# XunshanMan/MVGFormer

Measured on AMD Instinct MI355X. Metric: decoder samples/sec (5-view, 1024 queries, 4 layers), higher is better.
Workload: dtype bf16; 1 GPU; cfg2: 5 views, 1024 queries x 15 joints, 4 decoder layers, maps [(128, 240), (64, 120), (32, 60)] x 256ch, all queries valid; parallelism=single GPU, pyramid_handoff=NCHW fp32 (reference producer format), packed per step, initial_poses='sample_space' grid over the whole space (SURVEY 8(d)), samples_in_flight=1, samples_per_forward=1, hip_graph=True, device=gfx950:sramecc+:xnack-, cus=256

## Files before the change

### include/mvg_decoder.h

```cpp
#ifndef MVG_DECODER_H
#define MVG_DECODER_H

#include <stddef.h>
#include <stdint.h>

#ifdef __cplusplus
extern "C" {
#endif

#define MVG_F32 0
#define MVG_BF16 1

#define MVG_E_BADARG 10001
#define MVG_E_NOGPU 10002

#define MVG_CAM_STRIDE 48

int mvg_device_info(char* arch_out, int arch_len, int* cu_count);
const char* mvg_version(void);
int mvg_set_tuning(const char* key, int value);

int mvg_msda_forward_f32(const float* value, const int64_t* spatial_shapes,
                         const int64_t* level_start_index, const float* sampling_loc,
                         const float* attn_weight, float* out,
// ... 74 lines not shown
int mvg_msda_fused(const void* value, int dtype, const float* oa, const float* ref_lvl,
                   const int64_t* shapes_host, const int64_t* starts_host, void* samp,
                   int N_img, int Lq, int L, int S, void* stream);

int mvg_msda_gfused_f32(const float* value, const float* G, const float* xw, const float* ref_lvl,
                        const int64_t* shapes_host, const int64_t* starts_host, float* samp,
                        const uint8_t* pair_mask, const int32_t* order,
                        int N_img, int Lq, int L, int S, int B, void* stream);

int mvg_pyramid_group_ws(const void* feat, int n_img, int S, int njobs, const void* const* Wf, const float* const* bias,
                         void* const* out, const int* N, const int* planes, int slots_per_xcd, void* stream);
int mvg_msda_gsamp(const void* vh, const void* G, const float* xw, const float* ref_lvl,
                   const int64_t* shapes_host, const int64_t* starts_host, void* samp,
                   const uint8_t* pair_mask, const int32_t* order,
                   int N_img, int Lq, int L, int S, int B, void* stream);

size_t mvg_bin_pairs_workspace(int N_img, int Lq);
int mvg_bin_pairs(const float* ref_lvl, const uint8_t* inside, const int64_t* shapes_host, int L, int32_t* order,
                  int N_img, int Lq, void* workspace, size_t workspace_bytes, void* stream);

int mvg_mean_views(const void* attn, int dtype, void* out, int V, int rows, int C, void* stream);

int mvg_add_layernorm(const float* res, const void* h, int h_dtype, const float* gamma,
                      const float* beta, float* y, int rows, int C, void* stream);

int mvg_class_head(const float* tgt, const float* Wc, const float* bc, float threshold,
                   const uint8_t* forced_valid, float* prob, uint8_t* valid, int* any_valid,
                   int B, int NQ, int J, int C, void* stream);

int mvg_rowdot3(const void* h, int h_dtype, const float* W3, const float* b3, float* o,
                int rows, int C, void* stream);

int mvg_chain_attn_pose(const void* samp, const uint8_t* inside, const void* Wp, const float* bp,
                        const void* W0, const float* b0, const void* W1, const float* b1,
// ... 109 lines not shown
```

### mvgformer_amd/_lib.py

```python
from __future__ import annotations

import ctypes as C
import os

import torch

_HERE = os.path.dirname(os.path.abspath(__file__))
LIB_PATH = os.environ.get("MVG_LIB") or os.path.join(_HERE, "libmvgformer_hip.so")

MVG_F32, MVG_BF16 = 0, 1
CAM_STRIDE = 48

_vp, _i, _f = C.c_void_p, C.c_int, C.c_float

SIGNATURES = {
    "mvg_device_info": [C.c_char_p, _i, C.POINTER(_i)],
    "mvg_set_tuning": [C.c_char_p, _i],
    "mvg_msda_forward_f32": [_vp] * 6 + [_i] * 7 + [_vp],
    "mvg_msda_forward_bf16": [_vp] * 6 + [_i] * 7 + [_vp],
    "mvg_msda_backward_f32": [_vp] * 9 + [_i] * 7 + [_vp],
    "mvg_msda_backward_det_workspace": [_i] * 7 + [_vp],
    "mvg_msda_backward_det_f32": [_vp] * 9 + [_i] * 7 + [_vp, C.c_size_t, _vp],
    "mvg_msda_backward_det_bf16": [_vp] * 9 + [_i] * 7 + [_vp, C.c_size_t, _vp],
    "mvg_msda_backward_bal_workspace": [_i] * 7 + [_vp, _i],
# ... 9 lines not shown
    "mvg_dlt_backward": [_vp, _vp, _vp, _vp, _vp, _vp, _vp, _i, _i, _i, _i, _vp],
    "mvg_linear_wgrad_bias_f32": [_vp, _i, _vp, _i, _vp, _vp, _vp, _vp, _i, _i, _i, _i, _vp],
    "mvg_linear_wgrad_bias_bf16": [_vp, _i, _vp, _i, _vp, _vp, _vp, _vp, _i, _i, _i, _i, _vp],
    "mvg_linear_ordered": [_vp, _i, _vp, _vp, _vp, _i, _vp, _i, _i, _i, _i, _vp, _vp, _vp, _vp],
    "mvg_linear_sum": [_vp, _vp, _i, _i, _vp, _i, _vp, _vp, _i, _i, _vp, _i, _i, _i, _i, _vp],
    "mvg_msda_fused": [_vp, _i, _vp, _vp, _vp, _vp, _vp, _i, _i, _i, _i, _vp],
    "mvg_msda_gfused_f32": [_vp] * 9 + [_i] * 5 + [_vp],
    "mvg_chain_attn_pose": [_vp] * 14 + [_i, _vp],
    "mvg_chain_update_ffn_class": [_vp, _i] + [_vp] * 13 + [_f] + [_vp] * 9 + [_i] * 5 + [_vp, _vp],
    "mvg_chain_update_ffn_class_f32h": [_vp, _i, _vp, _vp, _i, _vp, _vp, _vp, _vp, _i, _vp, _vp, _i, _vp, _vp, _vp, _vp, _vp, C.c_float, _vp,
                                        _vp, _vp, _vp, _vp, _vp, _vp, _i, _vp, _vp, _i, _i, _i, _i, _i, _vp],
    "mvg_chain_attn_pose_f32h": [_vp, _vp, _vp, _i, _vp, _vp, _i, _vp, _vp, _i, _vp, _vp, _vp, _vp, _vp, _vp, _vp, _i, _vp],
    "mvg_pyramid_f32h": [_vp, _vp, _i, _vp, _vp, _i, _vp, _vp, C.c_int64, _i, _vp],
    "mvg_pyramid_group_ws": [_vp, _i, _i, _i, _vp, _vp, _vp, _vp, _vp, _i, _vp],
    "mvg_msda_gsamp": [_vp] * 9 + [_i] * 5 + [_vp],
    "mvg_bin_pairs": [_vp] * 3 + [_i] + [_vp] + [_i] * 2 + [_vp, C.c_size_t, _vp],
    "mvg_bin_pairs_workspace": [_i, _i],
    "mvg_mean_views": [_vp, _i, _vp, _i, _i, _i, _vp],
    "mvg_add_layernorm": [_vp, _vp, _i, _vp, _vp, _vp, _i, _i, _vp],
    "mvg_class_head": [_vp, _vp, _vp, _f, _vp, _vp, _vp, _vp, _i, _i, _i, _i, _vp],
    "mvg_rowdot3": [_vp, _i, _vp, _vp, _vp, _i, _i, _vp],
    "mvg_triangulate": [_vp] * 8 + [_i] * 4 + [_vp],
    "mvg_triangulate_project": [_vp] * 8 + [_i] * 4 + [_vp, _i] + [_vp] * 4,
    "mvg_uncrop_undistort_jac": [_vp, _vp, _vp, _vp, _i, _i, _i, _vp],
    "mvg_sym4_eigh": [_vp] * 3 + [C.c_long, _vp],
    "mvg_knn_match_workspace": [_i] * 3,
    "mvg_knn_match": [_vp, _vp, _vp, _i, _vp, _vp, _i, _i, _f] + [_i] * 5 + [_vp, C.c_size_t] + [_vp] * 5,
    "mvg_knn_match_jm": [_vp, _vp, _vp, _i, _vp, _vp, _i, _i, _f] + [_i] * 5 + [_vp, _i, _vp, C.c_size_t] + [_vp] * 5,
    "mvg_criterion_workspace": [_i] * 5,
    "mvg_criterion": [_vp] * 10 + [_i] + [_vp] * 4 + [_f] * 3 + [_i] * 7 + [_vp, C.c_size_t] + [_vp] * 5,
    "mvg_criterion_jm": [_vp] * 10 + [_i] + [_vp] * 4 + [_f] * 3 + [_i] * 5 + [_vp] + [_i] * 3 + [_vp, C.c_size_t] + [_vp] * 5,
# ... 91 lines not shown
```

### mvgformer_amd/csrc/geom.hip

```cpp
#include "common.h"

template <typename T>
__device__ __forceinline__ void pack_tile(const float* __restrict__ src, T* __restrict__ feat, int C, int HW, int S, int start,
                                          int bx, float (&tile)[64][65]) {
  const int n = blockIdx.z, tid = threadIdx.x;
  const int hw0 = bx * 64, c0 = blockIdx.y * 64;
  const int tx = tid & 63, ty = tid >> 6;
  const float* sp = src + (long)n * C * HW;
  float v[16];
#pragma unroll
  for (int i = 0; i < 16; ++i) {
    const int c = min(c0 + ty + 4 * i, C - 1), hw = min(hw0 + tx, HW - 1);
    v[i] = sp[(long)c * HW + hw];
  }
#pragma unroll
  for (int i = 0; i < 16; ++i) tile[ty + 4 * i][tx] = v[i];
  __syncthreads();
  T* fp = feat + ((long)n * S + start) * C;
  const int cq = tid & 15, p = tid >> 4, c = c0 + 4 * cq;
  const bool vec = (C & 3) == 0;
#pragma unroll
  for (int i = 0; i < 4; ++i) {
    const int hw = hw0 + p + 16 * i;
    if (hw >= HW || c >= C) continue;
// ... 768 lines not shown

constexpr int BIN_BITS = 6, BIN_KEYS = 1 << (2 * BIN_BITS);

__device__ __forceinline__ unsigned spread1(unsigned v) {
  v &= 0x3fu;
  v = (v | (v << 8)) & 0x00ff00ffu;
  v = (v | (v << 4)) & 0x0f0f0f0fu;
  v = (v | (v << 2)) & 0x33333333u;
  v = (v | (v << 1)) & 0x55555555u;
  return v;
}

template <int KPT>
__global__ __launch_bounds__(1024) void bin_pairs_kernel(const float* __restrict__ ref_lvl,
                                                         const uint8_t* __restrict__ inside, int* __restrict__ order,
                                                         int Lq, int L, int W0, int H0, int shift) {
  __shared__ int hist[BIN_KEYS + 1];
  __shared__ int wave_tot[16];
  const int n = blockIdx.x, tid = threadIdx.x;
  for (int i = tid; i <= BIN_KEYS; i += 1024) hist[i] = 0;
  float rx[KPT], ry[KPT];
  uint8_t in[KPT];
#pragma unroll
  for (int k = 0; k < KPT; ++k) {
    const long pair = (long)n * Lq + min(tid + 1024 * k, Lq - 1);
    const float2 rr = *reinterpret_cast<const float2*>(ref_lvl + pair * L * 2);
    rx[k] = rr.x;
    ry[k] = rr.y;
    in[k] = inside ? inside[pair] : (uint8_t)1;
  }
  __syncthreads();
  int key[KPT];
#pragma unroll
  for (int k = 0; k < KPT; ++k) {
    const int cx = min(max((int)(fminf(fmaxf(rx[k], 0.f), 1.f) * (float)W0), 0), W0 - 1) >> shift;
    const int cy = min(max((int)(fminf(fmaxf(ry[k], 0.f), 1.f) * (float)H0), 0), H0 - 1) >> shift;
    key[k] = in[k] ? (int)(spread1((unsigned)cx) | (spread1((unsigned)cy) << 1)) : BIN_KEYS;
    const bool live = tid + 1024 * k < Lq;
    const unsigned long long outm = __ballot(live && key[k] == BIN_KEYS);
    if (live && key[k] != BIN_KEYS) atomicAdd(&hist[key[k]], 1);
    if (outm && (tid & 63) == 0) atomicAdd(&hist[BIN_KEYS], __popcll(outm));
  }
  __syncthreads();
  const int c0 = hist[4 * tid], c1 = hist[4 * tid + 1], c2 = hist[4 * tid + 2], c3 = hist[4 * tid + 3];
  const int mine = c0 + c1 + c2 + c3;
  int incl = mine;
#pragma unroll
  for (int d = 1; d < 64; d <<= 1) {
    const int up = __shfl_up(incl, d, 64);
    if ((tid & 63) >= d) incl += up;
  }
  if ((tid & 63) == 63) wave_tot[tid >> 6] = incl;
  __syncthreads();
  int base = 0, total = 0;
#pragma unroll
  for (int w = 0; w < 16; ++w) {
    const int t = wave_tot[w];
    base += (w < (tid >> 6)) ? t : 0;
    total += t;
  }
  __syncthreads();
  const int ex = base + incl - mine;
  hist[4 * tid] = ex;
  hist[4 * tid + 1] = ex + c0;
  hist[4 * tid + 2] = ex + c0 + c1;
  hist[4 * tid + 3] = ex + c0 + c1 + c2;
  if (tid == 0) hist[BIN_KEYS] = total;
  __syncthreads();
#pragma unroll
  for (int k = 0; k < KPT; ++k) {
    const bool live = tid + 1024 * k < Lq;
    const bool out = live && key[k] == BIN_KEYS;
    const unsigned long long outm = __ballot(out);
    int pos = 0;
    if (live && !out) pos = atomicAdd(&hist[key[k]], 1);
    int obase = 0;
    if (outm && (tid & 63) == 0) obase = atomicAdd(&hist[BIN_KEYS], __popcll(outm));
    obase = __shfl(obase, 0, 64);
    if (out) pos = obase + __popcll(outm & ((1ull << (tid & 63)) - 1ull));
    if (live) order[(long)n * Lq + pos] = n * Lq + tid + 1024 * k;
  }
}

int g_bin_multi = 1;
constexpr int BIN_PARTS = 8;
constexpr int BIN_MULTI_MIN = 8192;
constexpr int BIN_CNT_STRIDE = BIN_KEYS + 4;

template <int KPT>
__global__ __launch_bounds__(1024) void bin_count_kernel(const float* __restrict__ ref_lvl,
                                                         const uint8_t* __restrict__ inside, unsigned* __restrict__ cnt,
                                                         unsigned short* __restrict__ keys_out, int Lq, int Lp, int L,
                                                         int W0, int H0, int shift) {
  __shared__ int hist[BIN_KEYS + 4];
  const int n = blockIdx.x / BIN_PARTS, part = blockIdx.x % BIN_PARTS, tid = threadIdx.x;
// ... 18 lines not shown
    const bool live = tid + 1024 * k < nq;
    const unsigned long long outm = __ballot(live && key == BIN_KEYS);
    if (live && key != BIN_KEYS) atomicAdd(&hist[key], 1);
    if (outm && (tid & 63) == 0) atomicAdd(&hist[BIN_KEYS], __popcll(outm));
    if (live) keys_out[(long)n * Lq + q0 + tid + 1024 * k] = (unsigned short)key;
  }
  __syncthreads();
  unsigned* dst = cnt + (long)blockIdx.x * BIN_CNT_STRIDE;
  *reinterpret_cast<uint4*>(dst + 4 * tid) = *reinterpret_cast<const uint4*>(&hist[4 * tid]);
  if (tid == 0) *reinterpret_cast<uint4*>(dst + BIN_KEYS) = *reinterpret_cast<const uint4*>(&hist[BIN_KEYS]);
}

template <int KPT>
__global__ __launch_bounds__(1024) void bin_scatter_kernel(const unsigned* __restrict__ cnt,
                                                           const unsigned short* __restrict__ keys_in,
                                                           int* __restrict__ order, int Lq, int Lp) {
  __shared__ int hist[BIN_KEYS + 4];
  __shared__ int wave_tot[16];
  __shared__ int out_sums[2];
  const int n = blockIdx.x / BIN_PARTS, part = blockIdx.x % BIN_PARTS, tid = threadIdx.x;
  const int n_img = gridDim.x / BIN_PARTS;
  constexpr int OVN = 16;
  int ov[OVN];
  if (tid < 64) {
#pragma unroll
    for (int j = 0; j < OVN; ++j) {
      const int i = tid + 64 * j;
      ov[j] = i < n_img * BIN_PARTS ? (int)cnt[(long)i * BIN_CNT_STRIDE + BIN_KEYS] : 0;
    }
  }
  const int q0 = part * Lp, nq = max(0, min(Lp, Lq - q0));
// ... 30 lines not shown
      ob += ((tid + 64 * j) / BIN_PARTS < n) ? ov[j] : 0;
    }
    for (int i = tid + 64 * OVN; i < n_img * BIN_PARTS; i += 64) {
      const int v = (int)cnt[(long)i * BIN_CNT_STRIDE + BIN_KEYS];
      oa += v;
      ob += (i / BIN_PARTS < n) ? v : 0;
    }
#pragma unroll
    for (int off = 32; off > 0; off >>= 1) {
      ob += __shfl_xor(ob, off, 64);
      oa += __shfl_xor(oa, off, 64);
    }
    if (tid == 0) {
      out_sums[0] = ob;
      out_sums[1] = oa;
    }
  }
  __syncthreads();
  int base = 0, total = 0;
#pragma unroll
  for (int w = 0; w < 16; ++w) {
    const int t = wave_tot[w];
    base += (w < (tid >> 6)) ? t : 0;
    total += t;
  }
  const int ex = base + incl - mine;
  hist[4 * tid] = ex + before[0];
  hist[4 * tid + 1] = ex + tot[0] + before[1];
  hist[4 * tid + 2] = ex + tot[0] + tot[1] + before[2];
  hist[4 * tid + 3] = ex + tot[0] + tot[1] + tot[2] + before[3];
// ... 307 lines not shown
  int e = mvg_fill_levels(&lv, shapes_host, zeros, L);
  if (e) return e;
  const long total = (long)V * B * Lq;
  if (total == 0) return 0;
  hipLaunchKernelGGL(project_kernel, dim3(mvg_ceil_div(total, 256)), dim3(256), 0, (hipStream_t)stream, X, cams, lv, r,
                     ref_lvl, inside, B, Lq, total);
  MVG_LAUNCH_CHECK();
  return 0;
}

size_t mvg_bin_pairs_workspace(int N_img, int Lq) {
  if (N_img <= 0 || Lq < BIN_MULTI_MIN) return 0;
  return (size_t)N_img * BIN_PARTS * BIN_CNT_STRIDE * sizeof(unsigned) + (size_t)N_img * Lq * sizeof(unsigned short);
}

int mvg_bin_pairs(const float* ref_lvl, const uint8_t* inside, const int64_t* shapes_host, int L, int32_t* order,
                  int N_img, int Lq, void* workspace, size_t workspace_bytes, void* stream) {
  if (!ref_lvl || !shapes_host || !order || L <= 0 || N_img < 0 || Lq < 0) return MVG_E_BADARG;
  if ((long)N_img * Lq > 0x7fffffffL) return MVG_E_BADARG;
  if (N_img == 0 || Lq == 0) return 0;
  const int H0 = (int)shapes_host[0], W0 = (int)shapes_host[1];
  if (H0 <= 0 || W0 <= 0) return MVG_E_BADARG;
  int shift = 2;
  while (((W0 - 1) >> shift) >= (1 << BIN_BITS) || ((H0 - 1) >> shift) >= (1 << BIN_BITS)) ++shift;
  if (Lq > 64 * 1024) return MVG_E_BADARG;
  hipStream_t st = (hipStream_t)stream;
  if (g_bin_multi && Lq >= BIN_MULTI_MIN && workspace && workspace_bytes >= mvg_bin_pairs_workspace(N_img, Lq)) {
    unsigned* cnt = reinterpret_cast<unsigned*>(workspace);
    unsigned short* keys = reinterpret_cast<unsigned short*>(cnt + (size_t)N_img * BIN_PARTS * BIN_CNT_STRIDE);
    const int Lp = ((Lq + BIN_PARTS - 1) / BIN_PARTS + 63) / 64 * 64;
#define MVG_BIN2(K)                                                                                              \
  {                                                                                                              \
    hipLaunchKernelGGL((bin_count_kernel<K>), dim3(N_img * BIN_PARTS), dim3(1024), 0, st, ref_lvl, inside, cnt,  \
                       keys, Lq, Lp, L, W0, H0, shift);                                                          \
    hipLaunchKernelGGL((bin_scatter_kernel<K>), dim3(N_img * BIN_PARTS), dim3(1024), 0, st, cnt, keys,           \
                       (int*)order, Lq, Lp);                                                                     \
  }
    if (Lp <= 1024) MVG_BIN2(1)
    else if (Lp <= 2 * 1024) MVG_BIN2(2)
    else if (Lp <= 4 * 1024) MVG_BIN2(4)
    else MVG_BIN2(8)
#undef MVG_BIN2
    MVG_LAUNCH_CHECK();
    return 0;
  }
#define MVG_BIN(K)                                                                                               \
  hipLaunchKernelGGL((bin_pairs_kernel<K>), dim3(N_img), dim3(1024), 0, st, ref_lvl, inside,                     \
                     (int*)order, Lq, L, W0, H0, shift)
  if (Lq <= 2 * 1024) MVG_BIN(2);
  else if (Lq <= 4 * 1024) MVG_BIN(4);
  else if (Lq <= 8 * 1024) MVG_BIN(8);
  else if (Lq <= 16 * 1024) MVG_BIN(16);
  else if (Lq <= 32 * 1024) MVG_BIN(32);
  else MVG_BIN(64);
#undef MVG_BIN
  MVG_LAUNCH_CHECK();
  return 0;
}

int mvg_gather_ref(const void* feat, int dtype, const float* ref_lvl, const float* x, const int64_t* shapes_host,
                   const int64_t* starts_host, void* ain, int V, int B, int Lq, int L, int S, int C, void* stream) {
  if (!feat || !ref_lvl || !x || !shapes_host || !starts_host || !ain || C % 4 != 0) return MVG_E_BADARG;
  LevelTable lv;
  int e = mvg_fill_levels(&lv, shapes_host, starts_host, L);
  if (e) return e;
  const long pairs = (long)V * B * Lq;
  if (pairs == 0) return 0;
  const int grid = mvg_ceil_div(pairs, 4);
  if (dtype == MVG_F32)
    hipLaunchKernelGGL((gather_ref_kernel<float>), dim3(grid), dim3(256), 0, (hipStream_t)stream, (const float*)feat, ref_lvl, x,
                       lv, (float*)ain, B, Lq, S, C, (int)pairs);
  else if (dtype == MVG_BF16)
// ... 139 lines not shown
```

### mvgformer_amd/csrc/msda.hip

```cpp
#include <string.h>

#include "common.h"
#include "gsamp_dev.h"


template <typename T>
__device__ __forceinline__ f32x4 bilinear4(const T* __restrict__ lvl_base, int H, int W, long row_stride,
                                           float h_im, float w_im, float scale) {
  const bool inside = (h_im > -1.f) && (w_im > -1.f) && (h_im < (float)H) && (w_im < (float)W);
  h_im = index_safe(h_im, (float)H);
  w_im = index_safe(w_im, (float)W);
  const float hl_f = floorf(h_im), wl_f = floorf(w_im);
  const int h_low = (int)hl_f, w_low = (int)wl_f;
  const int h_high = h_low + 1, w_high = w_low + 1;
  const float lh = h_im - hl_f, lw = w_im - wl_f;
  const float hh = 1.f - lh, hw = 1.f - lw;
  const float s = inside ? scale : 0.f;
  const bool hl_ok = h_low >= 0, hh_ok = h_high <= H - 1, wl_ok = w_low >= 0, wh_ok = w_high <= W - 1;
  const float w1 = (hl_ok && wl_ok) ? hh * hw : 0.f;
  const float w2 = (hl_ok && wh_ok) ? hh * lw : 0.f;
  const float w3 = (hh_ok && wl_ok) ? lh * hw : 0.f;
  const float w4 = (hh_ok && wh_ok) ? lh * lw : 0.f;
  const int hl_c = min(max(h_low, 0), H - 1), hh_c = min(max(h_high, 0), H - 1);
  const int wl_c = min(max(w_low, 0), W - 1), wh_c = min(max(w_high, 0), W - 1);
// ... 721 lines not shown
  if (reset) {
    const unsigned z = 0;
    e = hipMemcpyToSymbol(HIP_SYMBOL(gsamp_stamp_count), &z, sizeof(z));
    if (e != hipSuccess) return -(int)e;
  }
  return (int)n;
}
#endif

template <int L, int NT, int PIPE = 0>
__device__ __forceinline__ void msda_gsamp_body(const bf16_t* __restrict__ vp, const bf16_t* __restrict__ G,
                                                const float* __restrict__ xw, const float* __restrict__ r,
                                                const LevelTable& lv, bf16_t* __restrict__ samp,
                                                const uint8_t* __restrict__ pair_mask,
                                                const int* __restrict__ order, int n_pairs,
                                                int Lq, int S, int B, int map_ch) {
  constexpr int SCP = 3 * L * 8 + 8;
  __shared__ __attribute__((aligned(16))) float scratch[NT / 64][16][SCP];
  const int wave = threadIdx.x >> 6, lane = threadIdx.x & 63;
  const int sub = lane & 3, pl = lane >> 2;
  int m, pblk;
  if (map_ch == 0) {
    m = blockIdx.x & 7;
    pblk = blockIdx.x >> 3;
  } else {
    const int xcd = blockIdx.x & 7, j = blockIdx.x >> 3;
    m = j & 7;
    const int t = j >> 3;
    pblk = ((t / map_ch) * 8 + xcd) * map_ch + t % map_ch;
  }
  const int slot = pblk * (NT / 4) + wave * 16 + pl;
#ifdef GSAMP_STAMPS
  const unsigned long long gs_t0 = __builtin_amdgcn_s_memrealtime();
  auto gs_flush = [&](bool sampled) {
    const unsigned long long act = __ballot(sampled);
    const int first = __ffsll((unsigned long long)__ballot(true)) - 1;
    if (wave == 0 && lane == first) {
      const unsigned s_ = atomicAdd(&gsamp_stamp_count, 1u);
      if (s_ < 65536) {
        unsigned hw, xcc;
        asm volatile("s_getreg_b32 %0, hwreg(HW_REG_HW_ID)" : "=s"(hw));
        asm volatile("s_getreg_b32 %0, hwreg(HW_REG_XCC_ID)" : "=s"(xcc));
        gsamp_stamps[s_ * 4] = blockIdx.x | ((unsigned long long)__popcll(act) << 32);
        gsamp_stamps[s_ * 4 + 1] = gs_t0;
// ... 21 lines not shown
    }
  }
  float acc[8];
  gsamp_unit<L, PIPE>(vp, G, xw, r, lv, &scratch[wave][pl][0], pair, m, sub, Lq, S, B, acc, mine);
  store_acc<bf16_t, 8>(samp + (long)pair * 256 + m * 32 + sub * 8, acc);
#ifdef GSAMP_STAMPS
  gs_flush(true);
#endif
}

template <int L, int NT>
__global__ __launch_bounds__(NT) void msda_gsamp_kernel(const bf16_t* __restrict__ vp, const bf16_t* __restrict__ G,
                                                        const float* __restrict__ xw, const float* __restrict__ r,
                                                        LevelTable lv, bf16_t* __restrict__ samp,
                                                        const uint8_t* __restrict__ pair_mask, const int* __restrict__ order,
                                                        int n_pairs, int Lq, int S, int B, int map_ch) {
  msda_gsamp_body<L, NT>(vp, G, xw, r, lv, samp, pair_mask, order, n_pairs, Lq, S, B, map_ch);
}
template <int L, int NT>
__global__ __launch_bounds__(NT) void msda_gsamp_pipe_kernel(const bf16_t* __restrict__ vp, const bf16_t* __restrict__ G,
                                                             const float* __restrict__ xw, const float* __restrict__ r,
                                                             LevelTable lv, bf16_t* __restrict__ samp,
                                                             const uint8_t* __restrict__ pair_mask, const int* __restrict__ order,
                                                             int n_pairs, int Lq, int S, int B, int map_ch) {
  msda_gsamp_body<L, NT, 1>(vp, G, xw, r, lv, samp, pair_mask, order, n_pairs, Lq, S, B, map_ch);
}

static int g_gsamp_pipe = 0;
int g_auto_small = 1;
static int g_gsamp_map = 4;
static int g_gfused_chunk = 4;
static int g_gsamp_lds_pad = 0;
static int g_gsamp_threads = 256;

template <typename T, int CPL, int NB>
static int launch_msda_fused_cpl(const T* value, const float* oa, const float* r, const LevelTable& lv, T* samp,
                                 int n_pairs, int Lq, int S, hipStream_t st) {
  constexpr int PPW = CPL / 4;
  const int grid = (n_pairs + 4 * PPW - 1) / (4 * PPW);
  switch (lv.L) {
// ... 180 lines not shown
    case 32: MVG_BWD(32); break;
    case 64: MVG_BWD(64); break;
    default: {
      hipError_t e = hipMemsetAsync(grad_sampling_loc, 0, sizeof(float) * (size_t)N * Lq * M * L * P * 2, st);
      if (e != hipSuccess) return (int)e;
      e = hipMemsetAsync(grad_attn_weight, 0, sizeof(float) * (size_t)N * Lq * M * L * P, st);
      if (e != hipSuccess) return (int)e;
      MVG_BWD(0);
    }
  }
#undef MVG_BWD
  MVG_LAUNCH_CHECK();
  return 0;
}

int mvg_msda_gsamp(const void* vp, const void* G, const float* xw, const float* ref_lvl, const int64_t* shapes_host,
                   const int64_t* starts_host, void* samp, const uint8_t* pair_mask, const int32_t* order, int N_img,
                   int Lq, int L, int S, int B, void* stream) {
  if (!vp || !G || !xw || !ref_lvl || !shapes_host || !starts_host || !samp || B <= 0) return MVG_E_BADARG;
  LevelTable lv;
  int e = mvg_fill_levels(&lv, shapes_host, starts_host, L);
  if (e) return e;
  const long pairs = (long)N_img * Lq;
  if (pairs > 0x7fffffffL / 4) return MVG_E_BADARG;
  if ((long)N_img * S * 384 >= 0xffffffffL || (long)N_img * 8 * S * 64 >= 0xffffffffL) return MVG_E_BADARG;
  if (pairs == 0) return 0;
  hipStream_t st = (hipStream_t)stream;
  const bool pipe = g_gsamp_pipe == 1 || (g_gsamp_pipe == 0 && (long)N_img * Lq >= 32768);
  int nthreads = g_gsamp_threads, map = g_gsamp_map;
  if (g_auto_small && Lq <= 8192) {
    nthreads = 128;
    map = 1;
  }
#define MVG_GS(LL, NT)                                                                                            \
  {                                                                                                               \
    int npb = (int)((pairs + NT / 4 - 1) / (NT / 4));                                                             \
    if (map > 0) npb = (npb + 8 * map - 1) / (8 * map) * (8 * map);                                               \
    if (pipe)                                                                                                 \
      hipLaunchKernelGGL((msda_gsamp_pipe_kernel<LL, NT>), dim3(8 * npb), dim3(NT), g_gsamp_lds_pad, st, (const bf16_t*)vp,     \
                         (const bf16_t*)G, xw, ref_lvl, lv, (bf16_t*)samp, pair_mask, order, (int)pairs, Lq, S,   \
                         B, map);                                                                                 \
    else                                                                                                          \
      hipLaunchKernelGGL((msda_gsamp_kernel<LL, NT>), dim3(8 * npb), dim3(NT), g_gsamp_lds_pad, st, (const bf16_t*)vp,          \
                         (const bf16_t*)G, xw, ref_lvl, lv, (bf16_t*)samp, pair_mask, order, (int)pairs, Lq, S,   \
                         B, map);                                                                                 \
  }
#define MVG_GSN(LL)                                                                                               \
  if (nthreads == 1024) MVG_GS(LL, 1024) else if (nthreads == 512) MVG_GS(LL, 512)                                \
  else if (nthreads == 128) MVG_GS(LL, 128) else MVG_GS(LL, 256)
  switch (L) {
    case 1: MVG_GSN(1); break;
    case 2: MVG_GSN(2); break;
    case 3: MVG_GSN(3); break;
    case 4: MVG_GSN(4); break;
    default: return MVG_E_BADARG;
  }
#undef MVG_GSN
#undef MVG_GS
  MVG_LAUNCH_CHECK();
  return 0;
}

extern int g_chain_rm;
extern int g_chain_a_lds_pad;
extern int g_linear_tiles;
extern int g_f32_split;
extern int g_wreg_grid;
extern int g_f32h_rows;
extern int g_bin_multi;

int mvg_set_tuning(const char* key, int value) {
  if (!key) return MVG_E_BADARG;
  if (!strcmp(key, "linear_tiles") && value >= 0 && value <= 2) { g_linear_tiles = value; return 0; }
  if (!strcmp(key, "f32_split") && (value == 0 || value == 1)) { g_f32_split = value; return 0; }
  if (!strcmp(key, "f32h_rows") && (value == 0 || value == 32 || value == 64)) { g_f32h_rows = value; return 0; }
// ... 60 lines not shown
```

### mvgformer_amd/decoder.py

```python
from __future__ import annotations

import copy
import os

import torch
import torch.nn.functional as F
from torch import nn

from . import ops
from .projattn import ProjAttn, WeightCache



class MLP(nn.Module):

    def __init__(self, input_dim, hidden_dim, output_dim, num_layers):
        super().__init__()
        self.num_layers = num_layers
        h = [hidden_dim] * (num_layers - 1)
        self.layers = nn.ModuleList(nn.Linear(n, k) for n, k in zip([input_dim] + h, h + [output_dim]))

    def forward(self, x):
        for i, layer in enumerate(self.layers):
            x = F.relu(layer(x)) if i < self.num_layers - 1 else layer(x)
# ... 148 lines not shown
        self.use_confidences = False
        self.class_embed = nn.Linear(d_model, 2)
        self.num_joints = num_joints
        self.feature_update_method = feature_update_method
        self.init_self_attention = init_self_attention
        self.open_forward_ffn = open_forward_ffn
        self.query_filter_method = query_filter_method
        self.visualization_jump_num = visualization_jump_num
        self.triangulation_method = triangulation_method
        self.filter_query = filter_query
        self.d_model = d_model
        self.compute_dtype = torch.float32
        self.training_dtype = torch.float32
        self.use_fused_chains = True
        self.use_fused_chains_f32 = os.environ.get("MVG_F32_FUSED", "1") != "0"
        self.fuse_boundary = True
        self.skip_masked_f32 = True
        self._wc = WeightCache()
        self._run = None
        self._any_valid_hook = None

    def set_compute_dtype(self, dtype):
        if dtype not in (torch.float32, torch.bfloat16):
            raise ValueError("compute dtype must be float32 or bfloat16")
        self.compute_dtype = dtype
        self.proj_attn.compute_dtype = dtype
        return self

    def set_training_dtype(self, dtype):
        if dtype not in (torch.float32, torch.bfloat16):
# ... 308 lines not shown
        if xw_in is not None and tuple(xw_in.shape) != (B * Lq, 192):
            xw_in = None
        f32 = torch.float32
        pose_layers = self.pose_embed.MLP.layers
        o = None
        if self.proj_attn._vp_event is None and getattr(ctx, "_packed_event", None) is not None:
            torch.cuda.current_stream().wait_event(ctx._packed_event)
            ctx.feat.record_stream(torch.cuda.current_stream())
        if path_a == "bf16":
            order = None
            mode = self.proj_attn.sort_pairs if Lq <= 65536 else False
            if mode == "first":
                if getattr(ctx, "order", None) is None or ctx.order.numel() != V * B * Lq:
                    ctx.order = ops.bin_pairs(ref_lvl, None, ctx.levels)
                order = ctx.order
            elif mode:
                order = ops.bin_pairs(ref_lvl, inside.view(-1), ctx.levels)
            samp = self.proj_attn.native_sample(x, ref_lvl, ctx.feat, ctx.levels, V, B, pair_mask=inside.view(-1),
                                                order=order, xw=xw_in)
            wts, o_masked = self._chain_a_weights(dt)
            attn, o = ops.chain_attn_pose(samp, inside.view(-1), *wts, order=order, o_masked=o_masked)
        elif path_a == "f32h":
            order = ops.bin_pairs(ref_lvl, inside.view(-1), ctx.levels) if (self.proj_attn.sort_pairs and Lq <= 65536) else None
            samp = self.proj_attn.native_sample(x, ref_lvl, ctx.feat, ctx.levels, V, B, pair_mask=inside.view(-1), order=order,
                                                xw=xw_in)
            wts, o_masked = self._chain_a_weights_f32h()
            attn, o = ops.chain_attn_pose_f32h(samp, inside.view(-1), *wts, order=order, o_masked=o_masked)
        else:
            order32 = None
            if (dt == torch.float32 and self.skip_masked_f32 and C == 256 and 8192 <= Lq <= 65536
                    and self.proj_attn.sort_pairs):
                order32 = ops.bin_pairs(ref_lvl, inside.view(-1), ctx.levels)
            attn = self.proj_attn.native_forward(x(), ref_lvl, ctx.feat, ctx.levels, V, B, rowmask=inside.view(-1), order=order32)

        forced = None
# ... 306 lines not shown
```

### mvgformer_amd/ops.py

```python
from __future__ import annotations

import ctypes as C

import math

import numpy as np
import torch

from . import _lib as L

BACKWARD_MODE = __import__("os").environ.get("MVG_BACKWARD", "det")
BACKWARD_CHUNK = None


def _det_entry(lib, bf16, dims, shapes_c):
    kind = "bf16" if bf16 else "f32"
    if BACKWARD_MODE == "balanced":
        chunk = 0 if BACKWARD_CHUNK is None else int(BACKWARD_CHUNK)
        if chunk < 0 or chunk % 256:
            raise L.MvgError("BACKWARD_CHUNK must be None, 0 or a positive multiple of 256 (got %r)" % (BACKWARD_CHUNK,))
        name = "mvg_msda_backward_bal_" + kind
        return getattr(lib, name), name, int(lib.mvg_msda_backward_bal_workspace(*dims, shapes_c, chunk)), (chunk,)
    name = "mvg_msda_backward_det_" + kind
    return getattr(lib, name), name, int(lib.mvg_msda_backward_det_workspace(*dims, shapes_c)), ()
# ... 396 lines not shown
def msda_gsamp(vp, G, xw, r, levels, B, pair_mask=None, order=None, out=None):
    n_img = vp.shape[0]
    Lq = r.shape[1]
    samp = out if out is not None else torch.empty((n_img * Lq, 256), dtype=torch.bfloat16, device=vp.device)
    assert samp.dtype == torch.bfloat16 and tuple(samp.shape) == (n_img * Lq, 256) and samp.is_contiguous()
    if pair_mask is not None:
        assert pair_mask.dtype == torch.uint8 and pair_mask.numel() == n_img * Lq and pair_mask.is_contiguous()
    if order is not None:
        assert order.dtype == torch.int32 and order.numel() == n_img * Lq and order.is_contiguous()
    with _timed("msda_gsamp"):
      L.check(L.load().mvg_msda_gsamp(L.ptr(vp), L.ptr(G), L.ptr(xw), L.ptr(r), levels.shapes_c, levels.starts_c,
                                      L.ptr(samp), None if pair_mask is None else L.ptr(pair_mask),
                                      None if order is None else L.ptr(order), n_img, Lq, levels.L, levels.S, B,
                                      L.stream_ptr()), "mvg_msda_gsamp")
    return samp


def bin_pairs(r, inside, levels, out=None):
    n_img, Lq = r.shape[0], r.shape[1]
    if Lq > 65536:
        return None
    if out is None:
        out = torch.empty((n_img * Lq,), dtype=torch.int32, device=r.device)
    order = out
    lib = L.load()
    ws_bytes = int(lib.mvg_bin_pairs_workspace(n_img, Lq))
    ws = torch.empty((ws_bytes,), dtype=torch.uint8, device=r.device) if ws_bytes else None
    with _timed("bin_pairs"):
      L.check(lib.mvg_bin_pairs(L.ptr(r), None if inside is None else L.ptr(inside), levels.shapes_c, levels.L,
                                L.ptr(order), n_img, Lq, None if ws is None else L.ptr(ws), ws_bytes, L.stream_ptr()),
# ... 558 lines not shown
```

### mvgformer_amd/projattn.py

```python
from __future__ import annotations

import math
import warnings

import os

import torch
import torch.nn.functional as F
from torch import nn
from torch.nn.init import constant_, xavier_uniform_

from . import ops
from .functions import DeformFunction


def ops_host_levels_pair(spatial_shapes, level_start_index):
    sc, st = ops.host_levels(spatial_shapes, level_start_index)
    return [[sc[2 * i], sc[2 * i + 1]] for i in range(len(st))], list(st)


def _is_power_of_2(n):
    if (not isinstance(n, int)) or (n < 0):
        raise ValueError("invalid input for _is_power_of_2: {} (type: {})".format(n, type(n)))
    return (n & (n - 1) == 0) and n != 0
# ... 256 lines not shown
                self._wc.get("Woa_f32h", (self.sampling_offsets.weight, self.attention_weights.weight), f16, perm))

    def query_term_weights_f32h(self):
        Wpl = self.pyramid_planes_f32h()[1]
        perm = lambda a, b: torch.cat([a, b], 0)[ops.gsamp_column_order(a.device)]
        bpad = lambda a, b: torch.cat([perm(a, b), a.new_zeros(64)], 0)
        bn = self._wc.get("boa_pad", (self.sampling_offsets.bias, self.attention_weights.bias), torch.float32, bpad)
        return Wpl, bn, 192

    def _fast_query_weights(self, dt):
        perm = lambda a, b: torch.cat([a, b], 0)[ops.gsamp_column_order(a.device)]
        W = self._wc.get("Woa_perm", (self.sampling_offsets.weight, self.attention_weights.weight), dt, perm)
        b = self._wc.get("boa_perm", (self.sampling_offsets.bias, self.attention_weights.bias), torch.float32, perm)
        return W, b

    def native_sample(self, x, r, feat, levels, V, B, pair_mask=None, order=None, xw=None):
        dt = feat.dtype
        Wv, bv, Woa, boa, Wp, bp = self.weights(dt)
        n_img, S, Cc = feat.shape
        parts = getattr(x, "parts", None)
        f32_g = dt == torch.float32 and Cc == 256 and self.f32_g_form(r.shape[1], levels.L, S)
        if callable(x) and not (self.uses_fast_path(dt) and (xw is not None or parts is not None)) and not (f32_g and xw is not None):
            x = x()
        if self.uses_fast_path(dt):
            if order is None and self.sort_pairs and r.shape[1] <= 65536:
                order = ops.bin_pairs(r, pair_mask, levels)
            if xw is None:
                Wq, bq = self._fast_query_weights(dt)
                if parts is not None:
                    xw = ops.linear(parts[0].reshape(-1, Cc), Wq, bq, out_dtype=torch.float32, add=parts[1].reshape(-1, Cc))
                else:
                    xw = ops.linear(x.reshape(-1, Cc), Wq, bq, out_dtype=torch.float32)
            vp, G = self.project_pyramid(feat) if self._vp_event is None else self._wait_pyramid()
            return ops.msda_gsamp(vp, G, xw, r, levels, B, pair_mask=pair_mask, order=order)
        if f32_g:
            if xw is not None:
                xw32 = xw
            else:
                Wq, bq = self._fast_query_weights(dt)
                if callable(x):
                    x = x()
                xw32 = ops.linear(x.reshape(-1, Cc), Wq, bq, out_dtype=dt)
            if order is None and self.sort_pairs and r.shape[1] <= 65536:
                order = ops.bin_pairs(r, pair_mask, levels)
            value, G32 = self.project_pyramid(feat) if self._vp_event is None else self._wait_pyramid()
            return ops.msda_gfused_f32(value, G32, xw32, r, levels, B, pair_mask=pair_mask, order=order)
        ain = ops.gather_ref(feat, r, x, levels, V, B)
        oa = ops.linear(ain, Woa, boa, out_dtype=torch.float32)
        value = ops.linear(feat.view(n_img * S, Cc), Wv, bv, out_dtype=dt)
# ... 96 lines not shown
```

Baseline: 890.5 samples/s.

## Compact live view-query pairs globally and skip dead blocks in G-sampling

The pair-binning kernels now place every in-view pair, across all images, at the front of the global order and write the live count to a device scalar. A new gsamp_live entry point reads that scalar, and whole blocks past the live range return early, so dead pairs in out-of-view tails are never sampled. This is enabled automatically for large query counts on the bf16 fast path in non-first layers. In exchange, each binning block now scans the whole inside mask to compute prefix sums, and the first layer no longer requests a sort order.

```diff
diff --git a/include/mvg_decoder.h b/include/mvg_decoder.h
--- a/include/mvg_decoder.h
+++ b/include/mvg_decoder.h
@@ -112,10 +112,16 @@
                    const int64_t* shapes_host, const int64_t* starts_host, void* samp,
                    const uint8_t* pair_mask, const int32_t* order,
                    int N_img, int Lq, int L, int S, int B, void* stream);
+int mvg_msda_gsamp_live(const void* vh, const void* G, const float* xw, const float* ref_lvl,
+                        const int64_t* shapes_host, const int64_t* starts_host, void* samp,
+                        const uint8_t* pair_mask, const int32_t* order, const int32_t* n_live,
+                        int N_img, int Lq, int L, int S, int B, void* stream);
 
 size_t mvg_bin_pairs_workspace(int N_img, int Lq);
 int mvg_bin_pairs(const float* ref_lvl, const uint8_t* inside, const int64_t* shapes_host, int L, int32_t* order,
                   int N_img, int Lq, void* workspace, size_t workspace_bytes, void* stream);
+int mvg_bin_pairs_live(const float* ref_lvl, const uint8_t* inside, const int64_t* shapes_host, int L, int32_t* order,
+                       int32_t* n_live, int N_img, int Lq, void* workspace, size_t workspace_bytes, void* stream);
 
 int mvg_mean_views(const void* attn, int dtype, void* out, int V, int rows, int C, void* stream);
 
diff --git a/mvgformer_amd/_lib.py b/mvgformer_amd/_lib.py
--- a/mvgformer_amd/_lib.py
+++ b/mvgformer_amd/_lib.py
@@ -47,7 +47,9 @@
     "mvg_pyramid_f32h": [_vp, _vp, _i, _vp, _vp, _i, _vp, _vp, C.c_int64, _i, _vp],
     "mvg_pyramid_group_ws": [_vp, _i, _i, _i, _vp, _vp, _vp, _vp, _vp, _i, _vp],
     "mvg_msda_gsamp": [_vp] * 9 + [_i] * 5 + [_vp],
+    "mvg_msda_gsamp_live": [_vp] * 10 + [_i] * 5 + [_vp],
     "mvg_bin_pairs": [_vp] * 3 + [_i] + [_vp] + [_i] * 2 + [_vp, C.c_size_t, _vp],
+    "mvg_bin_pairs_live": [_vp] * 3 + [_i] + [_vp] * 2 + [_i] * 2 + [_vp, C.c_size_t, _vp],
     "mvg_bin_pairs_workspace": [_i, _i],
     "mvg_mean_views": [_vp, _i, _vp, _i, _i, _i, _vp],
     "mvg_add_layernorm": [_vp, _vp, _i, _vp, _vp, _vp, _i, _i, _vp],
diff --git a/mvgformer_amd/csrc/geom.hip b/mvgformer_amd/csrc/geom.hip
--- a/mvgformer_amd/csrc/geom.hip
+++ b/mvgformer_amd/csrc/geom.hip
@@ -806,11 +806,23 @@
 template <int KPT>
 __global__ __launch_bounds__(1024) void bin_pairs_kernel(const float* __restrict__ ref_lvl,
                                                          const uint8_t* __restrict__ inside, int* __restrict__ order,
-                                                         int Lq, int L, int W0, int H0, int shift) {
+                                                         int Lq, int L, int W0, int H0, int shift,
+                                                         int* __restrict__ n_live) {
   __shared__ int hist[BIN_KEYS + 1];
   __shared__ int wave_tot[16];
+  __shared__ int live_sums[2];
   const int n = blockIdx.x, tid = threadIdx.x;
   for (int i = tid; i <= BIN_KEYS; i += 1024) hist[i] = 0;
+  int lv_before = 0, lv_all = 0;
+  if (n_live) {
+    if (tid < 2) live_sums[tid] = 0;
+    const long n_all = (long)gridDim.x * Lq, mine0 = (long)n * Lq;
+    for (long i = tid; i < n_all; i += 1024) {
+      const int v = inside ? (inside[i] != 0) : 1;
+      lv_all += v;
+      lv_before += (i < mine0) ? v : 0;
+    }
+  }
   float rx[KPT], ry[KPT];
   uint8_t in[KPT];
 #pragma unroll
@@ -833,6 +845,17 @@
     if (live && key[k] != BIN_KEYS) atomicAdd(&hist[key[k]], 1);
     if (outm && (tid & 63) == 0) atomicAdd(&hist[BIN_KEYS], __popcll(outm));
   }
+  if (n_live) {
+#pragma unroll
+    for (int off = 32; off > 0; off >>= 1) {
+      lv_before += __shfl_xor(lv_before, off, 64);
+      lv_all += __shfl_xor(lv_all, off, 64);
+    }
+    if ((tid & 63) == 0) {
+      atomicAdd(&live_sums[0], lv_before);
+      atomicAdd(&live_sums[1], lv_all);
+    }
+  }
   __syncthreads();
   const int c0 = hist[4 * tid], c1 = hist[4 * tid + 1], c2 = hist[4 * tid + 2], c3 = hist[4 * tid + 3];
   const int mine = c0 + c1 + c2 + c3;
@@ -859,6 +882,12 @@
   hist[4 * tid + 3] = ex + c0 + c1 + c2;
   if (tid == 0) hist[BIN_KEYS] = total;
   __syncthreads();
+  long in_base = (long)n * Lq, out_base = (long)n * Lq;
+  if (n_live) {
+    in_base = live_sums[0];
+    out_base = (long)live_sums[1] + ((long)n * Lq - live_sums[0]) - total;
+    if (n == 0 && tid == 0) *n_live = live_sums[1];
+  }
 #pragma unroll
   for (int k = 0; k < KPT; ++k) {
     const bool live = tid + 1024 * k < Lq;
@@ -870,7 +899,7 @@
     if (outm && (tid & 63) == 0) obase = atomicAdd(&hist[BIN_KEYS], __popcll(outm));
     obase = __shfl(obase, 0, 64);
     if (out) pos = obase + __popcll(outm & ((1ull << (tid & 63)) - 1ull));
-    if (live) order[(long)n * Lq + pos] = n * Lq + tid + 1024 * k;
+    if (live) order[(out ? out_base : in_base) + pos] = n * Lq + tid + 1024 * k;
   }
 }
 
@@ -919,7 +948,8 @@
 template <int KPT>
 __global__ __launch_bounds__(1024) void bin_scatter_kernel(const unsigned* __restrict__ cnt,
                                                            const unsigned short* __restrict__ keys_in,
-                                                           int* __restrict__ order, int Lq, int Lp) {
+                                                           int* __restrict__ order, int Lq, int Lp,
+                                                           int* __restrict__ n_live) {
   __shared__ int hist[BIN_KEYS + 4];
   __shared__ int wave_tot[16];
   __shared__ int out_sums[2];
@@ -980,6 +1010,7 @@
     if (tid == 0) {
       out_sums[0] = ob;
       out_sums[1] = oa;
+      if (n_live && blockIdx.x == 0) *n_live = n_img * Lq - oa;
     }
   }
   __syncthreads();
@@ -1317,8 +1348,8 @@
   return (size_t)N_img * BIN_PARTS * BIN_CNT_STRIDE * sizeof(unsigned) + (size_t)N_img * Lq * sizeof(unsigned short);
 }
 
-int mvg_bin_pairs(const float* ref_lvl, const uint8_t* inside, const int64_t* shapes_host, int L, int32_t* order,
-                  int N_img, int Lq, void* workspace, size_t workspace_bytes, void* stream) {
+static int launch_bin_pairs(const float* ref_lvl, const uint8_t* inside, const int64_t* shapes_host, int L, int32_t* order,
+                            int32_t* n_live, int N_img, int Lq, void* workspace, size_t workspace_bytes, void* stream) {
   if (!ref_lvl || !shapes_host || !order || L <= 0 || N_img < 0 || Lq < 0) return MVG_E_BADARG;
   if ((long)N_img * Lq > 0x7fffffffL) return MVG_E_BADARG;
   if (N_img == 0 || Lq == 0) return 0;
@@ -1337,7 +1368,7 @@
     hipLaunchKernelGGL((bin_count_kernel<K>), dim3(N_img * BIN_PARTS), dim3(1024), 0, st, ref_lvl, inside, cnt,  \
                        keys, Lq, Lp, L, W0, H0, shift);                                                          \
     hipLaunchKernelGGL((bin_scatter_kernel<K>), dim3(N_img * BIN_PARTS), dim3(1024), 0, st, cnt, keys,           \
-                       (int*)order, Lq, Lp);                                                                     \
+                       (int*)order, Lq, Lp, (int*)n_live);                                                       \
   }
     if (Lp <= 1024) MVG_BIN2(1)
     else if (Lp <= 2 * 1024) MVG_BIN2(2)
@@ -1349,7 +1380,7 @@
   }
 #define MVG_BIN(K)                                                                                               \
   hipLaunchKernelGGL((bin_pairs_kernel<K>), dim3(N_img), dim3(1024), 0, st, ref_lvl, inside,                     \
-                     (int*)order, Lq, L, W0, H0, shift)
+                     (int*)order, Lq, L, W0, H0, shift, (int*)n_live)
   if (Lq <= 2 * 1024) MVG_BIN(2);
   else if (Lq <= 4 * 1024) MVG_BIN(4);
   else if (Lq <= 8 * 1024) MVG_BIN(8);
@@ -1359,6 +1390,18 @@
 #undef MVG_BIN
   MVG_LAUNCH_CHECK();
   return 0;
+}
+
+int mvg_bin_pairs(const float* ref_lvl, const uint8_t* inside, const int64_t* shapes_host, int L, int32_t* order,
+                  int N_img, int Lq, void* workspace, size_t workspace_bytes, void* stream) {
+  return launch_bin_pairs(ref_lvl, inside, shapes_host, L, order, nullptr, N_img, Lq, workspace, workspace_bytes, stream);
+}
+
+int mvg_bin_pairs_live(const float* ref_lvl, const uint8_t* inside, const int64_t* shapes_host, int L, int32_t* order,
+                       int32_t* n_live, int N_img, int Lq, void* workspace, size_t workspace_bytes, void* stream) {
+  if (!n_live) return MVG_E_BADARG;
+  if (N_img == 0 || Lq == 0) return MVG_E_BADARG;
+  return launch_bin_pairs(ref_lvl, inside, shapes_host, L, order, n_live, N_img, Lq, workspace, workspace_bytes, stream);
 }
 
 int mvg_gather_ref(const void* feat, int dtype, const float* ref_lvl, const float* x, const int64_t* shapes_host,
diff --git a/mvgformer_amd/csrc/msda.hip b/mvgformer_amd/csrc/msda.hip
--- a/mvgformer_amd/csrc/msda.hip
+++ b/mvgformer_amd/csrc/msda.hip
@@ -759,7 +759,8 @@
                                                 const LevelTable& lv, bf16_t* __restrict__ samp,
                                                 const uint8_t* __restrict__ pair_mask,
                                                 const int* __restrict__ order, int n_pairs,
-                                                int Lq, int S, int B, int map_ch) {
+                                                int Lq, int S, int B, int map_ch,
+                                                const int* __restrict__ n_live) {
   constexpr int SCP = 3 * L * 8 + 8;
   __shared__ __attribute__((aligned(16))) float scratch[NT / 64][16][SCP];
   const int wave = threadIdx.x >> 6, lane = threadIdx.x & 63;
@@ -773,6 +774,10 @@
     m = j & 7;
     const int t = j >> 3;
     pblk = ((t / map_ch) * 8 + xcd) * map_ch + t % map_ch;
+  }
+  if (n_live) {
+    const int live_end = (*n_live + 255) & ~255;
+    if (pblk * (NT / 4) >= live_end) return;
   }
   const int slot = pblk * (NT / 4) + wave * 16 + pl;
 #ifdef GSAMP_STAMPS
@@ -824,16 +829,18 @@
                                                         const float* __restrict__ xw, const float* __restrict__ r,
                                                         LevelTable lv, bf16_t* __restrict__ samp,
                                                         const uint8_t* __restrict__ pair_mask, const int* __restrict__ order,
-                                                        int n_pairs, int Lq, int S, int B, int map_ch) {
-  msda_gsamp_body<L, NT>(vp, G, xw, r, lv, samp, pair_mask, order, n_pairs, Lq, S, B, map_ch);
+                                                        int n_pairs, int Lq, int S, int B, int map_ch,
+                                                        const int* __restrict__ n_live) {
+  msda_gsamp_body<L, NT>(vp, G, xw, r, lv, samp, pair_mask, order, n_pairs, Lq, S, B, map_ch, n_live);
 }
 template <int L, int NT>
 __global__ __launch_bounds__(NT) void msda_gsamp_pipe_kernel(const bf16_t* __restrict__ vp, const bf16_t* __restrict__ G,
                                                              const float* __restrict__ xw, const float* __restrict__ r,
                                                              LevelTable lv, bf16_t* __restrict__ samp,
                                                              const uint8_t* __restrict__ pair_mask, const int* __restrict__ order,
-                                                             int n_pairs, int Lq, int S, int B, int map_ch) {
-  msda_gsamp_body<L, NT, 1>(vp, G, xw, r, lv, samp, pair_mask, order, n_pairs, Lq, S, B, map_ch);
+                                                             int n_pairs, int Lq, int S, int B, int map_ch,
+                                                             const int* __restrict__ n_live) {
+  msda_gsamp_body<L, NT, 1>(vp, G, xw, r, lv, samp, pair_mask, order, n_pairs, Lq, S, B, map_ch, n_live);
 }
 
 static int g_gsamp_pipe = 0;
@@ -1044,9 +1051,9 @@
   return 0;
 }
 
-int mvg_msda_gsamp(const void* vp, const void* G, const float* xw, const float* ref_lvl, const int64_t* shapes_host,
-                   const int64_t* starts_host, void* samp, const uint8_t* pair_mask, const int32_t* order, int N_img,
-                   int Lq, int L, int S, int B, void* stream) {
+static int launch_msda_gsamp(const void* vp, const void* G, const float* xw, const float* ref_lvl, const int64_t* shapes_host,
+                             const int64_t* starts_host, void* samp, const uint8_t* pair_mask, const int32_t* order,
+                             const int32_t* n_live, int N_img, int Lq, int L, int S, int B, void* stream) {
   if (!vp || !G || !xw || !ref_lvl || !shapes_host || !starts_host || !samp || B <= 0) return MVG_E_BADARG;
   LevelTable lv;
   int e = mvg_fill_levels(&lv, shapes_host, starts_host, L);
@@ -1069,11 +1076,11 @@
     if (pipe)                                                                                                 \
       hipLaunchKernelGGL((msda_gsamp_pipe_kernel<LL, NT>), dim3(8 * npb), dim3(NT), g_gsamp_lds_pad, st, (const bf16_t*)vp,     \
                          (const bf16_t*)G, xw, ref_lvl, lv, (bf16_t*)samp, pair_mask, order, (int)pairs, Lq, S,   \
-                         B, map);                                                                                 \
+                         B, map, n_live);                                                                               \
     else                                                                                                          \
       hipLaunchKernelGGL((msda_gsamp_kernel<LL, NT>), dim3(8 * npb), dim3(NT), g_gsamp_lds_pad, st, (const bf16_t*)vp,          \
                          (const bf16_t*)G, xw, ref_lvl, lv, (bf16_t*)samp, pair_mask, order, (int)pairs, Lq, S,   \
-                         B, map);                                                                                 \
+                         B, map, n_live);                                                                               \
   }
 #define MVG_GSN(LL)                                                                                               \
   if (nthreads == 1024) MVG_GS(LL, 1024) else if (nthreads == 512) MVG_GS(LL, 512)                                \
@@ -1089,6 +1096,19 @@
 #undef MVG_GS
   MVG_LAUNCH_CHECK();
   return 0;
+}
+
+int mvg_msda_gsamp(const void* vp, const void* G, const float* xw, const float* ref_lvl, const int64_t* shapes_host,
+                   const int64_t* starts_host, void* samp, const uint8_t* pair_mask, const int32_t* order, int N_img,
+                   int Lq, int L, int S, int B, void* stream) {
+  return launch_msda_gsamp(vp, G, xw, ref_lvl, shapes_host, starts_host, samp, pair_mask, order, nullptr, N_img, Lq, L, S, B, stream);
+}
+
+int mvg_msda_gsamp_live(const void* vp, const void* G, const float* xw, const float* ref_lvl, const int64_t* shapes_host,
+                        const int64_t* starts_host, void* samp, const uint8_t* pair_mask, const int32_t* order,
+                        const int32_t* n_live, int N_img, int Lq, int L, int S, int B, void* stream) {
+  if (!pair_mask || !order || !n_live) return MVG_E_BADARG;
+  return launch_msda_gsamp(vp, G, xw, ref_lvl, shapes_host, starts_host, samp, pair_mask, order, n_live, N_img, Lq, L, S, B, stream);
 }
 
 extern int g_chain_rm;
diff --git a/mvgformer_amd/decoder.py b/mvgformer_amd/decoder.py
--- a/mvgformer_amd/decoder.py
+++ b/mvgformer_amd/decoder.py
@@ -186,6 +186,7 @@
         self.training_dtype = torch.float32
         self.use_fused_chains = True
         self.use_fused_chains_f32 = os.environ.get("MVG_F32_FUSED", "1") != "0"
+        self.gsamp_live = {"0": False, "1": True}.get(os.environ.get("MVG_GSAMP_LIVE", "auto"), "auto")
         self.fuse_boundary = True
         self.skip_masked_f32 = True
         self._wc = WeightCache()
@@ -524,11 +525,16 @@
                 if getattr(ctx, "order", None) is None or ctx.order.numel() != V * B * Lq:
                     ctx.order = ops.bin_pairs(ref_lvl, None, ctx.levels)
                 order = ctx.order
-            elif mode:
+            wts, o_masked = self._chain_a_weights(dt)
+            n_live = None
+            use_live = self.gsamp_live is True or (self.gsamp_live == "auto" and Lq >= ops.GSAMP_LIVE_MIN_LQ)
+            if (use_live and mode and mode != "first" and o_masked is not None and path_b == "bf16"
+                    and self.proj_attn.uses_fast_path(dt)):
+                order, n_live = ops.bin_pairs_live(ref_lvl, inside.view(-1), ctx.levels)
+            elif mode and mode != "first":
                 order = ops.bin_pairs(ref_lvl, inside.view(-1), ctx.levels)
             samp = self.proj_attn.native_sample(x, ref_lvl, ctx.feat, ctx.levels, V, B, pair_mask=inside.view(-1),
-                                                order=order, xw=xw_in)
-            wts, o_masked = self._chain_a_weights(dt)
+                                                order=order, xw=xw_in, n_live=n_live)
             attn, o = ops.chain_attn_pose(samp, inside.view(-1), *wts, order=order, o_masked=o_masked)
         elif path_a == "f32h":
             order = ops.bin_pairs(ref_lvl, inside.view(-1), ctx.levels) if (self.proj_attn.sort_pairs and Lq <= 65536) else None
diff --git a/mvgformer_amd/ops.py b/mvgformer_amd/ops.py
--- a/mvgformer_amd/ops.py
+++ b/mvgformer_amd/ops.py
@@ -434,6 +434,39 @@
                                       None if order is None else L.ptr(order), n_img, Lq, levels.L, levels.S, B,
                                       L.stream_ptr()), "mvg_msda_gsamp")
     return samp
+
+
+GSAMP_LIVE_MIN_LQ = 8192
+
+
+def msda_gsamp_live(vp, G, xw, r, levels, B, pair_mask, order, n_live, out=None):
+    n_img = vp.shape[0]
+    Lq = r.shape[1]
+    samp = out if out is not None else torch.empty((n_img * Lq, 256), dtype=torch.bfloat16, device=vp.device)
+    assert samp.dtype == torch.bfloat16 and tuple(samp.shape) == (n_img * Lq, 256) and samp.is_contiguous()
+    assert pair_mask.dtype == torch.uint8 and pair_mask.numel() == n_img * Lq and pair_mask.is_contiguous()
+    assert order.dtype == torch.int32 and order.numel() == n_img * Lq and order.is_contiguous()
+    assert n_live.dtype == torch.int32 and n_live.numel() == 1 and n_live.device == vp.device
+    with _timed("msda_gsamp"):
+      L.check(L.load().mvg_msda_gsamp_live(L.ptr(vp), L.ptr(G), L.ptr(xw), L.ptr(r), levels.shapes_c, levels.starts_c,
+                                           L.ptr(samp), L.ptr(pair_mask), L.ptr(order), L.ptr(n_live), n_img, Lq, levels.L,
+                                           levels.S, B, L.stream_ptr()), "mvg_msda_gsamp_live")
+    return samp
+
+
+def bin_pairs_live(r, inside, levels):
+    n_img, Lq = r.shape[0], r.shape[1]
+    assert 0 < Lq <= 65536 and n_img > 0
+    order = torch.empty((n_img * Lq,), dtype=torch.int32, device=r.device)
+    n_live = torch.empty((1,), dtype=torch.int32, device=r.device)
+    lib = L.load()
+    ws_bytes = int(lib.mvg_bin_pairs_workspace(n_img, Lq))
+    ws = torch.empty((ws_bytes,), dtype=torch.uint8, device=r.device) if ws_bytes else None
+    with _timed("bin_pairs"):
+      L.check(lib.mvg_bin_pairs_live(L.ptr(r), None if inside is None else L.ptr(inside), levels.shapes_c, levels.L,
+                                     L.ptr(order), L.ptr(n_live), n_img, Lq, None if ws is None else L.ptr(ws), ws_bytes,
+                                     L.stream_ptr()), "mvg_bin_pairs_live")
+    return order, n_live
 
 
 def bin_pairs(r, inside, levels, out=None):
diff --git a/mvgformer_amd/projattn.py b/mvgformer_amd/projattn.py
--- a/mvgformer_amd/projattn.py
+++ b/mvgformer_amd/projattn.py
@@ -294,7 +294,7 @@
         b = self._wc.get("boa_perm", (self.sampling_offsets.bias, self.attention_weights.bias), torch.float32, perm)
         return W, b
 
-    def native_sample(self, x, r, feat, levels, V, B, pair_mask=None, order=None, xw=None):
+    def native_sample(self, x, r, feat, levels, V, B, pair_mask=None, order=None, xw=None, n_live=None):
         dt = feat.dtype
         Wv, bv, Woa, boa, Wp, bp = self.weights(dt)
         n_img, S, Cc = feat.shape
@@ -312,7 +312,11 @@
                 else:
                     xw = ops.linear(x.reshape(-1, Cc), Wq, bq, out_dtype=torch.float32)
             vp, G = self.project_pyramid(feat) if self._vp_event is None else self._wait_pyramid()
+            if n_live is not None:
+                return ops.msda_gsamp_live(vp, G, xw, r, levels, B, pair_mask, order, n_live)
             return ops.msda_gsamp(vp, G, xw, r, levels, B, pair_mask=pair_mask, order=order)
+        if n_live is not None:
+            raise RuntimeError("native_sample: n_live is only taken by the bf16 G-sampling path")
         if f32_g:
             if xw is not None:
                 xw32 = xw
```

Result: no change. 898.6 samples/s, median of 6 (+0.9%).
